# AlexandraLJones/MCBRaT3D

Hardware: AMD Instinct MI355X
Metric: photons/sec (higher is better)
Workload: dtype f32/f64

## Files before the change

mcbrat3d_amd/csrc/mcbrat_blockwalk.hip:

```cpp
#include <float.h>

#include "mcbrat_device.h"

namespace mcbrat {

enum : int { BW_DEAD = 0, BW_MOVE = 1, BW_COLLIDE = 2, BW_SURFACE = 3, BW_TOP = 4, BW_CROSS = 5 };

__device__ __forceinline__ int locate_z(const double *ze, int nz, bool regular, double z0, double invDz, double z) {
  if (!regular) return find_cell(ze, nz, z);
  return min(max((int)((z - z0) * invDz), 0), nz - 1);
}
__device__ __forceinline__ int locate_near_uniform(const double *e, int n, double x0, double invCell, double v) {
  int i = min(max((int)((v - x0) * invCell), 0), n - 1);
  const double lo = e[i], hi = e[i + 1];
  i += (v >= hi && i < n - 1) ? 1 : 0;
  i -= (v < lo && i > 0) ? 1 : 0;
  return i;
}

__device__ __forceinline__ long long unwrapped_index(const double *e, int n, double x0, double L, double invL, double x) {
  const double k = floor((x - x0) * invL);
  return (long long)k * n + find_cell(e, n, x - k * L);
}

struct BlockLds {
  size_t slab, cursor, rec, cdf, ext, ssa, cum, pfi, blockOf, tbl, total;
};
__host__ __device__ inline BlockLds block_lds_layout(int nx, int ny, int nz, int nc, size_t slabLen, int nBlocks, size_t tblFloats,
                                                      int optics = 0, bool cdfTop = false) {
  BlockLds L;
  const size_t nvox = (size_t)nx * ny * nz;
  const size_t nB4 = ((size_t)nBlocks + 3) & ~(size_t)3;
  size_t o = sizeof(double) * (size_t)(nx + ny + nz + 3);
  L.slab = o; o += sizeof(long long) * slabLen;
  L.cursor = o; o += 16;
  o = (o + 15) & ~(size_t)15;
  L.rec = o; o += 16 * (size_t)nBlocks;
  L.cdf = o; o += cdfTop ? sizeof(double) * ((size_t)nz + (size_t)ny * nz) : 0;
  L.ext = o; o += optics == 0 ? 4 * nvox : 4 * nB4;
  L.ssa = o; o += optics == 0 ? 4 * nvox * nc : (optics == 2 ? 4 * nB4 * nc : 0);
  L.cum = o; o += nc > 1 ? (optics == 0 ? 4 * nvox * nc : (optics == 2 ? 4 * nB4 * nc : 0)) : 0;
  L.pfi = o; o += optics == 0 ? 2 * ((nvox * nc + 1) & ~(size_t)1) : (optics == 2 ? 2 * nB4 * nc : 0);
  L.blockOf = o; o += 2 * ((nvox + 1) & ~(size_t)1);
  o = (o + 3) & ~(size_t)3;
  L.tbl = o; o += 4 * tblFloats;
  L.total = o;
  return L;
}

template <int BLOCK, bool TBL_LDS, bool DEBUG, bool EMIT, int SIMPLE, int OPT = 0>
__global__ void __launch_bounds__(BLOCK, BLOCK == 1024 ? 4 : (BLOCK > 512 ? BLOCK / 128 : MCBRAT_MIN_WAVES_PER_SIMD))
trace_block_kernel(const DevParams p) {
  constexpr bool NOY = SIMPLE == 2 && !DEBUG;
  constexpr bool NEAR = SIMPLE == 3;
  const bool xyRegular = NEAR ? false : (SIMPLE != 0 ? true : p.xyRegular != 0);
  const bool zRegular = NEAR ? false : (SIMPLE != 0 ? true : p.zRegular != 0);
  const int nc = SIMPLE != 0 ? 1 : p.nc;
  extern __shared__ __align__(16) unsigned char smem_raw[];
#ifdef MCBRAT_POISON
  for (unsigned i = threadIdx.x; i < p.ldsBytes / 4u; i += BLOCK) reinterpret_cast<unsigned *>(smem_raw)[i] = 0xffffffffu;
  __syncthreads();
#endif
  double *s_edge = reinterpret_cast<double *>(smem_raw);
  const int nEdges = p.nx + p.ny + p.nz + 3;
  const int ncol = p.nx * p.ny;
  const int nvox = ncol * p.nz;
  const int slabLen = (int)p.slabStride;
  const int slabsLen = p.unitsWide ? 2 * slabLen : slabLen;
  const bool cdfTop = EMIT && p.cdfTopLds != 0;
  const BlockLds lay = block_lds_layout(p.nx, p.ny, p.nz, nc, (size_t)slabsLen, p.nBlocks, TBL_LDS ? (size_t)p.tblTotalFloats : 0, OPT, cdfTop);
  const int nB4 = (p.nBlocks + 3) & ~3;
  long long *s_slab = reinterpret_cast<long long *>(smem_raw + lay.slab);
  unsigned *s_cursor = reinterpret_cast<unsigned *>(smem_raw + lay.cursor);
  uint4 *s_blockRec = reinterpret_cast<uint4 *>(smem_raw + lay.rec);
  float *s_ext = reinterpret_cast<float *>(smem_raw + lay.ext);
  double *s_cdfLevel = reinterpret_cast<double *>(smem_raw + lay.cdf);
  double *s_cdfRow = s_cdfLevel + p.nz;
  float *s_ssa = reinterpret_cast<float *>(smem_raw + lay.ssa);
  float *s_cum = reinterpret_cast<float *>(smem_raw + lay.cum);
  uint16_t *s_pfi = reinterpret_cast<uint16_t *>(smem_raw + lay.pfi);
  uint16_t *s_blockOf = reinterpret_cast<uint16_t *>(smem_raw + lay.blockOf);
  float *s_tbl = reinterpret_cast<float *>(smem_raw + lay.tbl);
  __shared__ int s_tblOffset[MCBRAT_MAX_COMPONENTS], s_tblNSteps[MCBRAT_MAX_COMPONENTS];
  __shared__ float s_tblInvN[MCBRAT_MAX_COMPONENTS];
  if (threadIdx.x < MCBRAT_MAX_COMPONENTS) {
    s_tblOffset[threadIdx.x] = p.tblOffset[threadIdx.x];
    s_tblNSteps[threadIdx.x] = p.tblNSteps[threadIdx.x];
    s_tblInvN[threadIdx.x] = p.tblInvN[threadIdx.x];
  }
  for (int i = threadIdx.x; i < nEdges; i += BLOCK) s_edge[i] = p.edges[i];
  if (TBL_LDS)
    for (int i = threadIdx.x; i < p.tblTotalFloats; i += BLOCK) s_tbl[i] = p.tables[i];
  for (int i = threadIdx.x; i < slabsLen; i += BLOCK) s_slab[i] = 0;
  if (threadIdx.x == 0) s_cursor[0] = 0;
  for (int i = threadIdx.x; i < p.nBlocks; i += BLOCK) s_blockRec[i] = p.blockRec[i];
  for (int i = threadIdx.x; i < nvox; i += BLOCK) s_blockOf[i] = p.blockOf[i];
  if (OPT == 0) {
    for (int i = threadIdx.x; i < nvox; i += BLOCK) s_ext[i] = p.ext[i];
    for (int i = threadIdx.x; i < nc * nvox; i += BLOCK) { s_ssa[i] = p.ssa[i]; s_pfi[i] = p.pfi[i]; }
    if (nc > 1)
      for (int i = threadIdx.x; i < nc * nvox; i += BLOCK) s_cum[i] = p.cum[i];
  } else {
    for (int i = threadIdx.x; i < p.nBlocks; i += BLOCK) s_ext[i] = p.blockExt[i];
    if (OPT == 2) {
      for (int i = threadIdx.x; i < nc * nB4; i += BLOCK) {
        const int k = i / nB4, b = i - k * nB4;
        if (b < p.nBlocks) { s_ssa[i] = p.blockSsa[k * p.nBlocks + b]; s_pfi[i] = p.blockPfi[k * p.nBlocks + b]; if (nc > 1) s_cum[i] = p.blockCum[k * p.nBlocks + b]; }
      }
    }
  }
  if (cdfTop) {
    const long long nxy = (long long)p.nx * p.ny;
    for (int i = threadIdx.x; i < p.nz; i += BLOCK) s_cdfLevel[i] = p.voxelCDF[((long long)p.nx - 1) + (long long)p.nx * (p.ny - 1) + nxy * i];
    for (int i = threadIdx.x; i < p.ny * p.nz; i += BLOCK) { const int k = i / p.ny, j = i - k * p.ny; s_cdfRow[i] = p.voxelCDF[((long long)p.nx - 1) + (long long)p.nx * j + nxy * k]; }
  }
  __syncthreads();
  auto cumAt = [&](int k, int cell) -> float { if constexpr (OPT == 0) return s_cum[k * nvox + cell]; else if constexpr (OPT == 1) return p.cum[k * nvox + cell]; else return s_cum[k * nB4 + s_blockOf[cell]]; };
  auto ssaAt = [&](int k, int cell) -> float { if constexpr (OPT == 0) return s_ssa[k * nvox + cell]; else if constexpr (OPT == 1) return p.ssa[k * nvox + cell]; else return s_ssa[k * nB4 + s_blockOf[cell]]; };
  auto pfiAt = [&](int k, int cell) -> int { if constexpr (OPT == 0) return (int)s_pfi[k * nvox + cell]; else if constexpr (OPT == 1) return (int)p.pfi[k * nvox + cell]; else return (int)s_pfi[k * nB4 + s_blockOf[cell]]; };
  auto extOfCell = [&](int cell) -> float { if constexpr (OPT == 0) return s_ext[cell]; else return s_ext[s_blockOf[cell]]; };
  const float *__restrict__ tbl = TBL_LDS ? s_tbl : p.tables;
  const int offY = p.nx + 1, offZ = p.nx + p.ny + 2;
  const double invDz = (double)p.nz / (p.zMax - p.z0);

  const int lane = threadIdx.x & (kWave - 1);
  const unsigned long long laneBelow = (1ull << lane) - 1ull;

  unsigned long long unitFirst = 0;
  unsigned unitCount = 0, unitSplit = 0;
  long long *unitSlab = nullptr;

  int state = BW_DEAD;
  bool more = true;
  int slabOff = 0;
  uint32_t idLo = 0, idHi = 0, event = 0;
  double px = 0, py = 0, pz = 0;
  float dx = 0, dy = 0, dz = 1;
  float ivx = 0, ivy = 0, ivz = 0;
  float tnx = 0, tny = 0, tnz = 0, tcur = 0;
  float acc = 0, tau = 0, w = 0, extCur = 0, uX = 0, uY = 0, uZ = 0;
  unsigned rx = 0, ry = 0, rz = 0;
  unsigned spans = 0;
  int nScat = 0, nLegs = 0;
  long long dbgX = 0, dbgY = 0;
  int dbgZ = 0;
  unsigned int cLegs = 0, cCross = 0, cColl = 0, cAbs = 0, cTop = 0, cSurf = 0, cKill = 0, cSurv = 0;
  unsigned long long wIters = 0, wCrossPhases = 0, wCrossLanes = 0, wEventLanes = 0, wLaunchPhases = 0, wSurfPhases = 0;

  auto countCrossings = [&](double x, double y, int kzEnd) {
    const long long ex = unwrapped_index(s_edge, p.nx, p.x0, p.Lx, p.invLx, x);
    const long long ey = unwrapped_index(s_edge + offY, p.ny, p.y0, p.Ly, p.invLy, y);
    cCross += (unsigned)(llabs(ex - dbgX) + llabs(ey - dbgY) + abs(kzEnd - dbgZ));
  };

  auto locX = [&](double xw, bool canLeave, bool force = false) {
    if (p.nx == 1 && !force) return 0;
    if (canLeave) {
      const double shift = floor((xw - p.x0) * p.invLx) * p.Lx;
      px -= shift; xw -= shift;
      if (DEBUG) dbgX -= (long long)rint(shift * p.invLx) * p.nx;
    }
    if (xyRegular) return min(max((int)((xw - p.x0) * p.invDX), 0), p.nx - 1);
    double o = 0.0;
    return locate_periodic(s_edge, p.nx, p.x0, p.Lx, p.invLx, p.invCellX, NEAR || p.xyNearUniform != 0, o, xw);
  };
  auto locY = [&](double yw, bool canLeave, bool force = false) {
    if (NOY) return 0;
    if (p.ny == 1 && !force) return 0;
    if (canLeave) {
      const double shift = floor((yw - p.y0) * p.invLy) * p.Ly;
      py -= shift; yw -= shift;
      if (DEBUG) dbgY -= (long long)rint(shift * p.invLy) * p.ny;
    }
    if (xyRegular) return min(max((int)((yw - p.y0) * p.invDY), 0), p.ny - 1);
    double o = 0.0;
    return locate_periodic(s_edge + offY, p.ny, p.y0, p.Ly, p.invLy, p.invCellY, NEAR || p.xyNearUniform != 0, o, yw);
  };
  auto inRange = [](int j, unsigned r) { return min(max(j, (int)(r & 0xffffu)), (int)(r >> 16) - 1); };
  const bool legacyNoClamp = (DEBUG || kTestBounds) && (p.legacyTies & 1) != 0, legacyMoveNaN = (DEBUG || kTestBounds) && (p.legacyTies & 2) != 0,
             legacyKeepSpans = (DEBUG || kTestBounds) && (p.legacyTies & 4) != 0;
  auto inRangeX = [&](int j, unsigned r) { return legacyNoClamp ? j : inRange(j, r); };
  auto enterBlock = [&](int ix, int iy, int iz) {
    const int cell = ix + p.nx * (iy + p.ny * iz);
    const unsigned blk = s_blockOf[cell];
    const uint4 rec = s_blockRec[blk];
    if constexpr (OPT == 0) extCur = s_ext[cell]; else extCur = s_ext[blk];
    rx = rec.x; rz = rec.z;
    if (!NOY) ry = rec.y;
    const int fx = dx >= 0.0f ? (int)(rx >> 16) : (int)(rx & 0xffffu);
    const int fy = NOY ? 0 : (dy >= 0.0f ? (int)(ry >> 16) : (int)(ry & 0xffffu));
    const int fz = dz >= 0.0f ? (int)(rz >> 16) : (int)(rz & 0xffffu);
    spans |= rec.w;
    tnx = ((rec.w & 1u) || ivx == 0.0f) ? FLT_MAX : (float)(s_edge[fx] - px) * ivx;
    tny = (NOY || (rec.w & 2u) || ivy == 0.0f) ? FLT_MAX : (float)(s_edge[offY + fy] - py) * ivy;
    tnz = ivz == 0.0f ? FLT_MAX : (float)(s_edge[offZ + fz] - pz) * ivz;
  };

  unsigned nCrossLeg = 0;
  unsigned nBadLane = 0;
  const unsigned maxEvents = (DEBUG || kTestBounds) ? p.maxEvents : kMaxEvents, maxEventsNaN = (DEBUG || kTestBounds) ? p.maxEventsNaN : kMaxEventsNaN,
                 watchdog = (DEBUG || kTestBounds) ? p.watchdog : kWatchdog;
#define MCBRAT_BW_DROP(kind_) do { \
    if constexpr (DEBUG || kTestBounds) record_first_drop(p.bad, (kind_), 2u, idLo, idHi, state, event);   \
    if (DEBUG && p.fates) p.fates[(((unsigned long long)idHi << 32) | idLo) - p.firstPhoton] = mcbrat_fate{3, 0, 0, 0, nScat, nLegs, w}; \
    state = BW_DEAD; \
    nBadLane = count_drop(nBadLane, (kind_));   \
  } while (0)
#ifdef MCBRAT_STAMPS
  __shared__ unsigned long long s_tprev[BLOCK / 64], s_stamp[BLOCK / 64][9];
  if (lane == 0) { s_tprev[threadIdx.x >> 6] = clock64(); for (int i = 0; i < 9; i++) s_stamp[threadIdx.x >> 6][i] = 0; }
#endif
  for (unsigned long long unit = blockIdx.x;; unit += gridDim.x) {
    if (unit >= p.nUnits) break;
    if (p.unitsWide) {
      const unsigned long long lo = p.total * unit / p.nUnits, hi = p.total * (unit + 1) / p.nUnits;
      const unsigned long long b = lo / p.ppb, end = (b + 1) * p.ppb;
      unitFirst = lo;
      unitCount = (unsigned)(hi - lo);
      unitSplit = (unsigned)((hi < end ? hi : end) - lo);
      unitSlab = p.slabs + b * p.slabStride;
    } else {
      const unsigned long long b = unit / p.unitsPerBatch, s = unit % p.unitsPerBatch;
      const unsigned long long bp = (p.total - b * p.ppb) < p.ppb ? (p.total - b * p.ppb) : p.ppb;
      const unsigned long long lo = (bp * s) / p.unitsPerBatch, hi = (bp * (s + 1)) / p.unitsPerBatch;
      unitFirst = b * p.ppb + lo;
      unitCount = (unsigned)(hi - lo);
      unitSplit = unitCount;
      unitSlab = p.slabs + b * p.slabStride;
    }
    more = true;

    for (;;) {
      bool needLeg = false;
      int ix = 0, iy = 0, iz = 0;

      const unsigned long long mSurf = __ballot(state == BW_SURFACE || state == BW_TOP);
      const unsigned long long mCross = __ballot(state == BW_CROSS);
      const int nBusy = __popcll(__ballot(state == BW_COLLIDE));
      const bool idle = nBusy < p.eventThreshold;
      const bool doSurface = __popcll(mSurf) >= p.surfaceThreshold || idle;
      const bool doCross = __popcll(mCross) >= p.crossThreshold || idle;
      if ((state == BW_SURFACE || state == BW_TOP) && doSurface) {
        const bool top = state == BW_TOP;
        {
          const double xw = px + (double)tcur * (double)dx, yw = py + (double)tcur * (double)dy;
          if (DEBUG) countCrossings(xw, yw, top ? p.nz : -1);
          px = xw;
          if (!NOY) py = yw;
          const int jx = locX(xw, true, true);
          ix = inRange(jx, rx);
          if (ix != jx) {
            const double lo = s_edge[rx & 0xffffu], hi = s_edge[rx >> 16];
            if (px < lo && lo - px > px + p.Lx - hi) px += p.Lx;
            else if (px > hi && px - hi > lo - (px - p.Lx)) px -= p.Lx;
          }
          iy = 0;
          if (!NOY) {
            const int jy = locY(yw, true, true);
            iy = inRange(jy, ry);
            if (iy != jy) {
              const double lo = s_edge[offY + (ry & 0xffffu)], hi = s_edge[offY + (ry >> 16)];
              if (py < lo && lo - py > py + p.Ly - hi) py += p.Ly;
              else if (py > hi && py - hi > lo - (py - p.Ly)) py -= p.Ly;
            }
          }
        }
        atomicAdd(reinterpret_cast<unsigned long long *>(s_slab + slabOff + (top ? 0 : ncol) + (ix + p.nx * iy)), weight_to_fixed(w));
        if (top) {
          if (DEBUG) {
            cTop++;
            if (p.fates) p.fates[(((unsigned long long)idHi << 32) | idLo) - p.firstPhoton] = mcbrat_fate{0, ix + 1, iy + 1, p.nz + 1, nScat, nLegs, w};
          }
          state = BW_DEAD;
        } else {
          pz = p.zSurf;
          iz = 0;
          nScat++;
          if (DEBUG) cSurf++;
          float mu = sqrtf(uX);
          if (!(fabsf(mu) > 2.0f * FLT_MIN)) {
            mu = sqrtf(uZ);
            uint32_t r[4];
            for (uint32_t j = 0; !(fabsf(mu) > 2.0f * FLT_MIN); j++) {
              if ((j & 3u) == 0) philox4x32_10(event, 2u + (j >> 2), idLo, idHi, p.seedLo, p.seedHi, r);
              mu = sqrtf(u01(pick4(r, j & 3u)));
            }
          }
          const float wIn = w;
          if (SIMPLE == 0 && p.surfNumX > 0) w = w * surface_reflectance(p, px, py);
          else w = (float)((double)w * (double)p.albedo);
          if (w <= FLT_MIN) {
            if (DEBUG && p.fates) p.fates[(((unsigned long long)idHi << 32) | idLo) - p.firstPhoton] = mcbrat_fate{1, ix + 1, iy + 1, 1, nScat, nLegs, wIn};
            state = BW_DEAD;
          } else {
            const float sinTheta = sqrtf(1.0f - mu * mu);
            float cphi, sphi;
            sincos_2pi(uY, cphi, sphi);
            dx = sinTheta * cphi; dy = sinTheta * sphi; dz = mu;
            needLeg = true;
          }
        }
      }
      STAMP(5);
      const unsigned long long mDead = __ballot(state == BW_DEAD && more);
      const bool doLaunch = __popcll(mDead) >= p.launchThreshold || idle;
      const unsigned long long want = doLaunch ? mDead : 0ull;
      if (DEBUG) {
        wIters++;
        wEventLanes += nBusy;
        if (want) wLaunchPhases++;
        if (doSurface && mSurf) wSurfPhases++;
        if (doCross && mCross) { wCrossPhases++; wCrossLanes += __popcll(mCross); }
      }
      if (want != 0ull) {
        const int nWant = __popcll(want);
        const int rank = __popcll(want & laneBelow);
        unsigned base = 0;
        if (lane == 0) base = atomicAdd(&s_cursor[0], (unsigned)nWant);
        base = (unsigned)__shfl((int)base, 0);
        const unsigned k = base + (unsigned)rank;
        const bool valid = k < unitCount;
        const unsigned long long myIdx = unitFirst + k;
        if (state == BW_DEAD && more) {
          if (valid) {
            const unsigned long long id = p.firstPhoton + myIdx;
            idLo = (uint32_t)id; idHi = (uint32_t)(id >> 32);
            event = 0; nScat = 0; nLegs = 0;
            slabOff = k < unitSplit ? 0 : slabLen;
            uint32_t r[4];
            philox4x32_10(0u, 0u, idLo, idHi, p.seedLo, p.seedHi, r);
            double lx, ly, lz;
            if (!EMIT) {
              lx = (double)u01(r[0]);
              ly = (double)u01(r[1]);
              lz = 0.0;
              dx = p.dir0[0]; dy = p.dir0[1]; dz = p.dir0[2];
            } else {
              float mu = 0.f, phi = 0.f;
              const float sel = u01(r[0]);
              if ((double)sel > p.fracAtms) {
                lx = (double)u01(r[1]);
                ly = (double)u01(r[2]);
                lz = 0.0;
                uint32_t r1[4];
                for (uint32_t j = 0;; j++) {
                  if ((j & 3u) == 0) philox4x32_10(0u, 1u + (j >> 2), idLo, idHi, p.seedLo, p.seedHi, r1);
                  mu = sqrtf(u01(pick4(r1, j & 3u)));
                  if (fabsf(mu) > 2.0f * FLT_MIN) break;
                }
                phi = (u01(r[3]) * 2.0f) * 3.14159274f;
              } else {
                const float rn = u01(r[1]);
                const long long nxy = (long long)p.nx * p.ny;
                const int ik = cdfTop ? find_cdf(s_cdfLevel, p.nz, 1, rn) : find_cdf(p.voxelCDF + ((long long)p.nx - 1) + (long long)p.nx * (p.ny - 1), p.nz, nxy, rn);
                const int ij = cdfTop ? find_cdf(s_cdfRow + p.ny * (ik - 1), p.ny, 1, rn) : find_cdf(p.voxelCDF + ((long long)p.nx - 1) + nxy * (ik - 1), p.ny, p.nx, rn);
                const int ii = find_cdf(p.voxelCDF + (long long)p.nx * ((ij - 1) + (long long)p.ny * (ik - 1)), p.nx, 1, rn);
                uint32_t r1[4];
                philox4x32_10(0u, 1u, idLo, idHi, p.seedLo, p.seedHi, r1);
                lz = ((double)(ik - 1) * 1.0 / (double)p.nz) + (double)(u01(r[2]) / (float)p.nz);
                if (ik == 1 && lz == 0.0) lz = 2.220446049250313e-16;
                if (ik == p.nz && lz > 1.0 - 2.0 * 2.220446049250313e-16) lz = lz - 2.0 * 2.220446049250313e-16;
                lx = ((double)(ii - 1) * 1.0 / (double)p.nx) + (double)(u01(r[3]) * (1.0f / (float)p.nx));
                ly = ((double)(ij - 1) * 1.0 / (double)p.ny) + (double)(u01(r1[0]) * (1.0f / (float)p.ny));
                uint32_t r2[4];
                for (uint32_t j = 0;; j++) {
                  uint32_t uu;
                  if (j < 2) uu = j ? r1[3] : r1[2];
                  else {
                    if (((j - 2) & 3u) == 0) philox4x32_10(0u, 2u + ((j - 2) >> 2), idLo, idHi, p.seedLo, p.seedHi, r2);
                    uu = pick4(r2, (j - 2) & 3u);
                  }
                  mu = 1.0f - (2.0f * u01(uu));
                  if (fabsf(mu) > 2.0f * FLT_MIN) break;
                }
                phi = (u01(r1[1]) * 2.0f) * 3.14159274f;
              }
              const float sinTheta = sqrtf(1.0f - mu * mu);
              dx = sinTheta * cosf(phi); dy = sinTheta * sinf(phi); dz = mu;
            }
            w = 1.0f;
            px = p.x0 + lx * (p.xMax - p.x0);
            if (!NOY) py = p.y0 + ly * (p.yMax - p.y0);
            if (xyRegular) {
              ix = min((int)((px - p.x0) * p.invDX), p.nx - 1);
              iy = NOY ? 0 : min((int)((py - p.y0) * p.invDY), p.ny - 1);
            } else {
              ix = NEAR ? locate_near_uniform(s_edge, p.nx, p.x0, p.invCellX, px) : find_cell(s_edge, p.nx, px);
              iy = NOY ? 0 : (NEAR ? locate_near_uniform(s_edge + offY, p.ny, p.y0, p.invCellY, py) : find_cell(s_edge + offY, p.ny, py));
            }
            if (!EMIT) {
              pz = p.zLaunch; iz = p.izLaunch;
            } else if (zRegular) {
              pz = p.z0 + lz * (p.zMax - p.z0);
              iz = min((int)((pz - p.z0) / ((p.zMax - p.z0) / (double)p.nz)), p.nz - 1);
            } else {
              const double t = (lz - p.z0) * (double)p.nz;
              const double fl = floor(t);
              iz = min((int)fl, p.nz - 1);
              pz = s_edge[offZ + iz] + (t - fl) * (s_edge[offZ + iz + 1] - s_edge[offZ + iz]);
            }
            if (EMIT && p.lwFlag && pz > 0.0)
              atomicAdd(reinterpret_cast<unsigned long long *>(s_slab + slabOff + 2 * ncol + (ix + p.nx * (iy + p.ny * iz))), to_fixed(-1.0));
            needLeg = true;
          } else {
            more = false;
          }
        }
      }
      STAMP(0);
      if (state == BW_COLLIDE) {
        if (dz == dz || legacyMoveNaN) {
          const double s = (double)(tcur + div_fast(tau - acc, extCur));
          px = px + s * (double)dx;
          if (!NOY) py = py + s * (double)dy;
          pz = pz + s * (double)dz;
        }
        {
          const double xw = px, yw = py;
          iz = NEAR ? locate_near_uniform(s_edge + offZ, p.nz, p.z0, invDz, pz) : locate_z(s_edge + offZ, p.nz, zRegular, p.z0, invDz, pz);
          ix = locX(xw, (spans & 1u) != 0);
          iy = locY(yw, (spans & 2u) != 0);
        }
        int cell = ix + p.nx * (iy + p.ny * iz);
        nScat++;
        if (DEBUG) cColl++;
        int c = 0;
        if (nc > 1) {
          for (int k = 0; k < nc - 1; k++)
            if (uZ >= cumAt(k, cell)) c = k + 1;
        }
        float ssa = ssaAt(c, cell);
        int pfEntry = pfiAt(c, cell);
        if (ssa <= 0.0f && extOfCell(cell) != extCur) {
          ix = inRange(ix, rx); iz = inRange(iz, rz);
          if (!NOY) iy = inRange(iy, ry);
          cell = ix + p.nx * (iy + p.ny * iz);
          c = 0;
          if (nc > 1) {
            for (int k = 0; k < nc - 1; k++)
              if (uZ >= cumAt(k, cell)) c = k + 1;
          }
          ssa = ssaAt(c, cell);
          pfEntry = pfiAt(c, cell);
        }
        if (DEBUG) countCrossings(px, py, iz);
        if (ssa < 1.0f) {
          atomicAdd(reinterpret_cast<unsigned long long *>(s_slab + slabOff + 2 * ncol + cell), weight_to_fixed(w * (1.0f - ssa)));
          w = w * ssa;
          if (DEBUG) cAbs++;
        }
        if (p.useRR && w < 0.5f) {
          float uR = uZ;
          if (nc != 1) {
            uint32_t r1[4];
            philox4x32_10(event, 1u, idLo, idHi, p.seedLo, p.seedHi, r1);
            uR = u01(r1[1]);
          }
          if (uR >= w) { w = 0.0f; if (DEBUG) cKill++; }
          else { w = 1.0f; if (DEBUG) cSurv++; }
        }
        STAMP(2);
        if (w <= FLT_MIN) {
          if (DEBUG && p.fates) p.fates[(((unsigned long long)idHi << 32) | idLo) - p.firstPhoton] = mcbrat_fate{2, ix + 1, iy + 1, iz + 1, nScat, nLegs, 0.0f};
          state = BW_DEAD;
        } else {
          const int n = s_tblNSteps[c];
          const float *t = tbl + s_tblOffset[c] + (long long)pfEntry * n;
          const int ai = (int)(uX * (float)n) + 1;
          float ang;
          if (ai < n) {
#ifdef MCBRAT_PRECISE_MATH
            const float left = uX - (float)(ai - 1) / (float)n;
#else
            const float left = uX - (float)(ai - 1) * s_tblInvN[c];
#endif
            ang = (1.0f - left) * t[ai - 1] + left * t[ai];
          } else {
            ang = t[n - 1];
          }
#ifdef MCBRAT_PRECISE_MATH
          const float cs = cosf(ang);
#else
          const float cs = cos_0_pi(ang);
#endif
          STAMP(3);
          float AX, AY;
          sincos_2pi(uY, AX, AY);
#ifdef MCBRAT_PRECISE_MATH
          float B = sqrtf(1.0f - cs * cs);
#else
          float B = __builtin_amdgcn_sqrtf(1.0f - cs * cs);
#endif
          AX = AX * B;
          AY = AY * B;
          B = dx * AX - dy * AY;
          float D = cs - div_fast(B, 1.0f + fabsf(dz));
          dx = dx * D + AX;
          dy = dy * D - AY;
          dz = dz * cs - copysignf(fabsf(B), dz * B);
          needLeg = true;
          STAMP(4);
        }
      }
      STAMP(4);
      if (needLeg && event >= maxEventsNaN) {
        if (event >= maxEvents || !(dz == dz || w < 1.0f)) { needLeg = false; MCBRAT_BW_DROP(event >= maxEvents ? DROP_LEGS : DROP_NAN_LEGS); }
      }
      if (needLeg) {
        event++;
        nLegs++;
        if (DEBUG) {
          cLegs++;
          dbgX = unwrapped_index(s_edge, p.nx, p.x0, p.Lx, p.invLx, px);
          dbgY = unwrapped_index(s_edge + offY, p.ny, p.y0, p.Ly, p.invLy, py);
          dbgZ = iz;
        }
        uint32_t r[4];
        philox4x32_10(event, 0u, idLo, idHi, p.seedLo, p.seedHi, r);
#ifdef MCBRAT_PRECISE_MATH
        tau = -logf(fmaxf(FLT_MIN, u01(r[0])));
#else
        tau = -0.693147182f * __builtin_amdgcn_logf(fmaxf(FLT_MIN, u01(r[0])));
#endif
        uX = u01(r[1]); uY = u01(r[2]); uZ = u01(r[3]);
        acc = 0.0f; tcur = 0.0f;
        ivx = fabsf(dx) >= 2.0f * FLT_MIN ? rcp_fast(dx) : 0.0f;
        ivy = (!NOY && fabsf(dy) >= 2.0f * FLT_MIN) ? rcp_fast(dy) : 0.0f;
        ivz = fabsf(dz) >= 2.0f * FLT_MIN ? rcp_fast(dz) : 0.0f;
        spans = 0;
        nCrossLeg = 0u;
        enterBlock(ix, iy, iz);
        state = BW_MOVE;
      }
      STAMP(6);
      if (state == BW_CROSS && doCross) {
        const bool yLtX = !NOY && tny < tnx;
        const float m2 = yLtX ? tny : tnx;
        const bool isZ = tnz < m2;
        const double xw = px + (double)tcur * (double)dx, yw = py + (double)tcur * (double)dy, zw = pz + (double)tcur * (double)dz;
        int jx, jy, jz;
        if (isZ) {
          jz = dz >= 0.0f ? (int)(rz >> 16) : (int)(rz & 0xffffu) - 1;
          jx = inRangeX(locX(xw, (spans & 1u) != 0), rx);
          jy = NOY ? 0 : inRangeX(locY(yw, (spans & 2u) != 0), ry);
        } else if (yLtX) {
          jy = dy >= 0.0f ? (int)(ry >> 16) : (int)(ry & 0xffffu) - 1;
          if (jy >= p.ny) { jy = 0; py -= p.Ly; if (DEBUG) dbgY -= p.ny; }
          else if (jy < 0) { jy = p.ny - 1; py += p.Ly; if (DEBUG) dbgY += p.ny; }
          jx = inRangeX(locX(xw, (spans & 1u) != 0), rx);
          jz = inRangeX(NEAR ? locate_near_uniform(s_edge + offZ, p.nz, p.z0, invDz, zw) : locate_z(s_edge + offZ, p.nz, zRegular, p.z0, invDz, zw), rz);
        } else {
          jx = dx >= 0.0f ? (int)(rx >> 16) : (int)(rx & 0xffffu) - 1;
          if (jx >= p.nx) { jx = 0; px -= p.Lx; if (DEBUG) dbgX -= p.nx; }
          else if (jx < 0) { jx = p.nx - 1; px += p.Lx; if (DEBUG) dbgX += p.nx; }
          jy = NOY ? 0 : inRangeX(locY(yw, (spans & 2u) != 0), ry);
          jz = inRangeX(NEAR ? locate_near_uniform(s_edge + offZ, p.nz, p.z0, invDz, zw) : locate_z(s_edge + offZ, p.nz, zRegular, p.z0, invDz, zw), rz);
        }
        if (!legacyKeepSpans) spans = 0;
        enterBlock(jx, jy, jz);
        state = BW_MOVE;
        if (++nCrossLeg > watchdog) MCBRAT_BW_DROP(DROP_CROSSINGS);
      }
      STAMP(1);
      if (__ballot(state != BW_DEAD || more) == 0ull) break;

#ifdef MCBRAT_STUCK_PROBE
      if (DEBUG && p.traceBuf && wIters > 3000000ull) {
        const unsigned long long live = __ballot(state != BW_DEAD);
        if (live != 0ull && lane == __ffsll((long long)live) - 1) {
          const unsigned long long r = wIters - 3000001ull;
          if (r < 64ull) {
            double *t = p.traceBuf + 20 * r;
            t[0] = 777; t[1] = state; t[2] = tcur; t[3] = tnx; t[4] = tny; t[5] = tnz; t[6] = (double)rx; t[7] = (double)ry; t[8] = (double)rz;
            t[9] = px; t[10] = py; t[11] = pz; t[12] = dx; t[13] = dy; t[14] = dz; t[15] = acc; t[16] = tau; t[17] = extCur; t[18] = spans; t[19] = idLo;
          } else {
            state = BW_DEAD;
          }
        }
      }
#endif
      if (state == BW_MOVE) {
        const bool yLtX = !NOY && tny < tnx;
        const float m2 = yLtX ? tny : tnx;
        const bool isZ = tnz < m2;
        const float tmin = isZ ? tnz : m2;
        const float accNew = acc + (tmin - tcur) * extCur;
        if (accNew > tau) {
          state = BW_COLLIDE;
        } else if (!(tmin < FLT_MAX)) {
          MCBRAT_BW_DROP(DROP_VACUUM);
        } else {
          acc = accNew;
          tcur = tmin;
          state = BW_CROSS;
          if (isZ && (dz >= 0.0f ? (int)(rz >> 16) == p.nz : (rz & 0xffffu) == 0u)) state = dz >= 0.0f ? BW_TOP : BW_SURFACE;
        }
      }
      STAMP(7);
    }

    __syncthreads();
    for (int i = threadIdx.x; i < slabsLen; i += BLOCK) {
      const long long v = s_slab[i];
      if (v != 0) {
        atomicAdd(reinterpret_cast<unsigned long long *>(unitSlab + i), (unsigned long long)v);
        s_slab[i] = 0;
      }
    }
    if (threadIdx.x == 0) s_cursor[0] = 0;
    __syncthreads();
  }

  publish_drops(p.bad, nBadLane);
#ifdef MCBRAT_STAMPS
  if (DEBUG && p.counters && lane == 0) for (int i = 0; i < 9; i++) atomicAdd(p.counters + 16 + i, s_stamp[threadIdx.x >> 6][i]);
#endif
  if (DEBUG && p.counters) {
    atomicAdd(p.counters + 0, (unsigned long long)cLegs);
    atomicAdd(p.counters + 1, (unsigned long long)cCross);
    atomicAdd(p.counters + 2, (unsigned long long)cColl);
    atomicAdd(p.counters + 3, (unsigned long long)cAbs);
    atomicAdd(p.counters + 4, (unsigned long long)cTop);
    atomicAdd(p.counters + 5, (unsigned long long)cSurf);
    atomicAdd(p.counters + 6, (unsigned long long)cKill);
    atomicAdd(p.counters + 7, (unsigned long long)cSurv);
    if (lane == 0) {
      atomicAdd(p.counters + 8, wCrossPhases); atomicAdd(p.counters + 9, wCrossLanes);
      atomicAdd(p.counters + 10, wIters); atomicAdd(p.counters + 11, wEventLanes);
      atomicAdd(p.counters + 12, wLaunchPhases); atomicAdd(p.counters + 13, wSurfPhases);
    }
  }
}

}
```

mcbrat3d_amd/csrc/mcbrat_kernels.hip:

```cpp
#include <float.h>

#include "mcbrat_device.h"

#ifdef MCBRAT_STAMPS
#define STAMP(i) do { if (DEBUG && p.counters) { const unsigned long long t_ = clock64(); \
    if (lane == __ffsll((long long)__ballot(1)) - 1) { s_stamp[threadIdx.x >> 6][i] += t_ - s_tprev[threadIdx.x >> 6]; s_tprev[threadIdx.x >> 6] = t_; } } } while (0)
#elif defined(MCBRAT_MARKS)
#define STAMP(i) asm volatile("; @@mark " #i)
#else
#define STAMP(i) do { } while (0)
#endif

namespace mcbrat {

constexpr unsigned kChunk = 256;
#ifndef MCBRAT_FLY_MIN_BRICKS
#define MCBRAT_FLY_MIN_BRICKS 8.0f
#endif
constexpr float kFlyMinBricks = MCBRAT_FLY_MIN_BRICKS;
constexpr int kWalkCap = 256;

#ifndef MCBRAT_MIN_WAVES_PER_SIMD
#define MCBRAT_MIN_WAVES_PER_SIMD 4
#endif
#ifndef MCBRAT_WAVES_GLOBAL_GRID
#define MCBRAT_WAVES_GLOBAL_GRID 6
#endif
#ifndef MCBRAT_WAVES_GLOBAL_GRID_INTEN
#define MCBRAT_WAVES_GLOBAL_GRID_INTEN 4
#endif

__device__ __forceinline__ uint32_t xor3(uint32_t a, uint32_t b, uint32_t c) {
#if defined(__gfx950__)
  return __builtin_amdgcn_bitop3_b32(a, b, c, 0x96);
#else
  return a ^ b ^ c;
#endif
}

__device__ __forceinline__ void philox4x32_10(uint32_t c0, uint32_t c1, uint32_t c2, uint32_t c3, uint32_t k0,
                                              uint32_t k1, uint32_t (&out)[4]) {
#pragma unroll
  for (int i = 0; i < 10; i++) {
    const unsigned long long p0 = (unsigned long long)0xD2511F53u * c0;
    const unsigned long long p1 = (unsigned long long)0xCD9E8D57u * c2;
    c0 = xor3((uint32_t)(p1 >> 32), c1, k0);
    c1 = (uint32_t)p1;
    c2 = xor3((uint32_t)(p0 >> 32), c3, k1);
    c3 = (uint32_t)p0;
    k0 += 0x9E3779B9u;
    k1 += 0xBB67AE85u;
  }
  out[0] = c0; out[1] = c1; out[2] = c2; out[3] = c3;
}

__device__ __forceinline__ float u01(uint32_t u) { return (float)u * 2.3283064365386963e-10f; }

#ifdef MCBRAT_PRECISE_MATH
__device__ __forceinline__ float rcp_fast(float x) { return 1.0f / x; }
__device__ __forceinline__ float div_fast(float a, float b) { return a / b; }
#else
__device__ __forceinline__ float rcp_fast(float x) { return __builtin_amdgcn_rcpf(x); }
__device__ __forceinline__ float div_fast(float a, float b) { return a * __builtin_amdgcn_rcpf(b); }
#endif

__device__ __forceinline__ float cos_0_pi(float x) {
  const float q = rintf(x * 0.636619772f);
  float r = __fmaf_rn(q, -1.57079637050628662109375f, x);
  r = __fmaf_rn(q, 4.371138828673793e-8f, r);
  const float z = r * r;
  const float c = __fmaf_rn(z, __fmaf_rn(z, __fmaf_rn(z, __fmaf_rn(z, 2.43904487962774090654e-5f, -1.38867637746099294692e-3f),
                                                      4.16666233237390631894e-2f), -0.499999997251031003120f), 1.0f);
  const float s = __fmaf_rn(r * z, __fmaf_rn(z, __fmaf_rn(z, __fmaf_rn(z, 2.7183114939898219064e-6f, -1.98393348360966317347e-4f),
                                                          8.3333293858894631756e-3f), -0.166666666416265235595f), r);
  return q == 0.0f ? c : (q == 1.0f ? -s : -c);
}

__device__ __forceinline__ void sincos_2pi(float u, float &c, float &s) {
  const float q = rintf(4.0f * u);
  const float r = (u - 0.25f * q) * 6.28318548202514648f;
  const float z = r * r;
  const float cc = __fmaf_rn(z, __fmaf_rn(z, __fmaf_rn(z, __fmaf_rn(z, 2.43904487962774090654e-5f, -1.38867637746099294692e-3f),
                                                       4.16666233237390631894e-2f), -0.499999997251031003120f), 1.0f);
  const float ss = __fmaf_rn(r * z, __fmaf_rn(z, __fmaf_rn(z, __fmaf_rn(z, 2.7183114939898219064e-6f, -1.98393348360966317347e-4f),
                                                           8.3333293858894631756e-3f), -0.166666666416265235595f), r);
  const int qi = (int)q & 3;
  c = qi == 0 ? cc : (qi == 1 ? -ss : (qi == 2 ? -cc : ss));
  s = qi == 0 ? ss : (qi == 1 ? cc : (qi == 2 ? -ss : -cc));
}

__device__ __forceinline__ uint32_t pick4(const uint32_t (&r)[4], uint32_t i) {
  const uint32_t a = (i & 1u) ? r[1] : r[0], b = (i & 1u) ? r[3] : r[2];
  return (i & 2u) ? b : a;
}

__device__ __forceinline__ unsigned long long to_fixed(double v) {
  return (unsigned long long)__double2ll_rn(v * kTallyScale);
}
__device__ __forceinline__ unsigned long long weight_to_fixed(float v) {
  return v >= 1.0f ? (1ull << 32) : (unsigned long long)__float2uint_rn(v * 4294967296.0f);
}

__device__ __forceinline__ int find_cell(const double *e, int n, double v) {
  int lo = 0, hi = n;
  while (hi - lo > 1) {
    const int mid = (lo + hi) >> 1;
    if (v >= e[mid]) lo = mid; else hi = mid;
  }
  return lo;
}

__device__ __forceinline__ int find_cdf(const double *t, int n, long long stride, float vf) {
  const double v = (double)vf;
  int lo = 0, hi = n;
  while (!(lo == n || hi <= lo + 1)) {
    const int mid = (lo + hi) >> 1;
    if (v > t[(long long)(mid - 1) * stride]) lo = mid; else hi = mid;
  }
  return hi;
}

__device__ __forceinline__ int locate_periodic(const double *e, int n, double x0, double L, double invL, double invCell,
                                               bool nearUniform, double &origin, double xw) {
  const double shift = floor((xw - x0) * invL) * L;
  origin -= shift;
  xw -= shift;
  if (!nearUniform) return find_cell(e, n, xw);
  int i = min(max((int)((xw - x0) * invCell), 0), n - 1);
  const double lo = e[i], hi = e[i + 1];
  i += (xw >= hi && i < n - 1) ? 1 : 0;
  i -= (xw < lo && i > 0) ? 1 : 0;
  return i;
}

__device__ __forceinline__ float make_periodic_f(double a, double aMin, double aMax) {
  float r = (float)a;
  for (int guard = 0; guard < 65536; ++guard) {
    if ((double)r <= aMax && (double)r > aMin) break;
    if ((double)r > aMax) r = (float)((double)r - (aMax - aMin));
    else if ((double)r == aMin) r = (float)aMax;
    else r = (float)((double)r + (aMax - aMin));
  }
  return r;
}
__device__ __forceinline__ int find_index_mixed(const double *t, int n, float vf) {
  const double v = (double)vf;
  int lo = 0, up = n;
  while (!(lo == n || up <= lo + 1)) {
    const int mid = (lo + up) >> 1;
    if (v >= t[mid - 1]) lo = mid; else up = mid;
  }
  return lo;
}
__device__ __forceinline__ float surface_reflectance(const DevParams &p, double x, double y) {
  const int xi = min(max(find_index_mixed(p.surfX, p.surfNumX, make_periodic_f(x, p.surfX[0], p.surfX[p.surfNumX - 1])), 1), p.surfNumX - 1);
  const int yi = min(max(find_index_mixed(p.surfY, p.surfNumY, make_periodic_f(y, p.surfY[0], p.surfY[p.surfNumY - 1])), 1), p.surfNumY - 1);
  return p.surfRefl[(xi - 1) + (p.surfNumX - 1) * (yi - 1)];
}

struct CellRef {
  int dense;
  int stored;
};

template <bool BRICK>
__device__ __forceinline__ CellRef locate_cell(const DevParams &p, int ix, int iy, int iz) {
  CellRef r;
  r.dense = ix + p.nx * (iy + p.ny * iz);
  r.stored = -1;
  if (BRICK) {
    const uint32_t base = p.brickTable[(ix >> 2) + p.nbx * ((iy >> 2) + p.nby * (iz >> 2))];
    if (base != 0xffffffffu) r.stored = (int)(base + (uint32_t)((ix & 3) + 4 * ((iy & 3) + 4 * (iz & 3))));
  }
  return r;
}

template <bool BRICK>
__device__ __forceinline__ float load_ext(const DevParams &p, const float *s_bgExt, const CellRef &r, int iz) {
  if (!BRICK) return p.extWalk[r.dense];
  return r.stored >= 0 ? p.ext[r.stored] : s_bgExt[iz];
}

template <int BLOCK, bool TBL_LDS, int PRIV, bool BRICK, bool DEBUG, bool INTEN = false, bool EMIT = true, int SPEC = 0>
__global__ void __launch_bounds__(BLOCK, BLOCK == 1024 ? 4 : BLOCK > 512 ? BLOCK / 128 : ((PRIV == 0 && !DEBUG) ? (INTEN ? MCBRAT_WAVES_GLOBAL_GRID_INTEN : MCBRAT_WAVES_GLOBAL_GRID) : MCBRAT_MIN_WAVES_PER_SIMD))
trace_kernel(const DevParams p) {
  constexpr int WALKSPEC = SPEC & 3, NCSPEC = (SPEC >> 2) & 3;
  static_assert(SPEC == 0 || WALKSPEC != 0, "the component count and the roulette are fixed in the walk-specialised instantiations only");
  const bool layerSkipOn = SPEC ? true : p.layerSkip != 0;
  const bool useRec = SPEC ? true : p.rec != nullptr;
  const bool xyRegularWalk = (WALKSPEC == 2 || WALKSPEC == 3) ? true : (WALKSPEC == 1 ? false : p.xyRegularWalk != 0);
  const bool zRegularWalk = WALKSPEC == 2 ? true : ((WALKSPEC == 1 || WALKSPEC == 3) ? false : p.zRegularWalk != 0);
  const bool surfaceDescription = SPEC ? false : p.surfNumX > 0;
  const int nc = NCSPEC ? NCSPEC : p.nc;
  const bool useRR = (SPEC & 16) ? true : p.useRR != 0;
  extern __shared__ __align__(16) unsigned char smem_raw[];
#ifdef MCBRAT_POISON
  for (unsigned i = threadIdx.x; i < p.ldsBytes / 4u; i += BLOCK) reinterpret_cast<unsigned *>(smem_raw)[i] = 0xffffffffu;
  __syncthreads();
#endif
  double *s_edge = reinterpret_cast<double *>(smem_raw);
  const int nEdges = p.nx + p.ny + p.nz + 3;
  const int offZ0 = p.nx + p.ny + 2;
  const int ncol = p.nx * p.ny;
  const int slabLen = PRIV ? (int)p.slabStride : 0;
  long long *s_slab = reinterpret_cast<long long *>(s_edge + nEdges);
  unsigned *s_cursor = reinterpret_cast<unsigned *>(s_slab + slabLen);
  float *s_bgExt = reinterpret_cast<float *>(s_cursor + (PRIV ? 4 : 0));
  constexpr bool gridLds = PRIV == 2;
  const int nvoxS = gridLds ? ncol * p.nz : 0;
  int *s_run = reinterpret_cast<int *>(s_bgExt + ((p.nz + 3) & ~3));
  double *s_runT = reinterpret_cast<double *>(s_run + ((p.nz + 3) & ~3));
  constexpr bool FLY = PRIV != 2 && !BRICK && !INTEN;
  const bool flyOn = FLY && (SPEC ? true : p.fly != 0);
  const int flyCols = FLY ? p.flyNbx * p.flyNby : 0;
  float *s_bgVal = reinterpret_cast<float *>(s_runT + ((p.nz + 2) & ~1));
  float2 *s_rangeZ = reinterpret_cast<float2 *>(s_bgVal + (flyCols ? ((p.nz + 3) & ~3) : 0));
  uint16_t *s_range = reinterpret_cast<uint16_t *>(s_rangeZ + flyCols);
  float *s_ext = reinterpret_cast<float *>(s_range + ((flyCols + 3) & ~3));
  float *s_ssa = s_ext + nvoxS;
  float *s_cum = s_ssa + (size_t)nc * nvoxS;
  uint16_t *s_pfi = reinterpret_cast<uint16_t *>(s_cum + (size_t)nc * nvoxS);
  float *s_tbl = reinterpret_cast<float *>(s_pfi + (((size_t)nc * nvoxS + 1) & ~(size_t)1));
  __shared__ int s_tblOffset[MCBRAT_MAX_COMPONENTS], s_tblNSteps[MCBRAT_MAX_COMPONENTS];
  __shared__ float s_tblInvN[MCBRAT_MAX_COMPONENTS];
  __shared__ int s_fwdOffset[MCBRAT_MAX_COMPONENTS], s_fwdNAngles[MCBRAT_MAX_COMPONENTS];
  __shared__ float s_flyTC[(PRIV != 2 && !BRICK && !INTEN) ? BLOCK : 1];
  if (INTEN && threadIdx.x < MCBRAT_MAX_COMPONENTS) {
    s_fwdOffset[threadIdx.x] = p.fwdOffset[threadIdx.x];
    s_fwdNAngles[threadIdx.x] = p.fwdNAngles[threadIdx.x];
  }
  if (threadIdx.x < MCBRAT_MAX_COMPONENTS) {
    s_tblOffset[threadIdx.x] = p.tblOffset[threadIdx.x];
    s_tblNSteps[threadIdx.x] = p.tblNSteps[threadIdx.x];
    s_tblInvN[threadIdx.x] = p.tblInvN[threadIdx.x];
  }
  for (int i = threadIdx.x; i < nEdges; i += BLOCK) s_edge[i] = p.edges[i];
  if (TBL_LDS)
    for (int i = threadIdx.x; i < p.tblTotalFloats; i += BLOCK) s_tbl[i] = p.tables[i];
  if (PRIV) {
    for (int i = threadIdx.x; i < slabLen; i += BLOCK) s_slab[i] = 0;
    if (threadIdx.x == 0) s_cursor[0] = 0;
  }
  for (int i = threadIdx.x; i < p.nz; i += BLOCK) { s_bgExt[i] = p.bgExt[i]; s_run[i] = p.layerRun[i]; }
  for (int i = threadIdx.x; i <= p.nz; i += BLOCK) s_runT[i] = p.layerRunT[i];
  if (FLY && flyCols) {
    for (int i = threadIdx.x; i < p.nz; i += BLOCK) s_bgVal[i] = p.bgVal[i];
    for (int i = threadIdx.x; i < flyCols; i += BLOCK) {
      const unsigned r = p.flyRange[i];
      s_range[i] = (uint16_t)r;
      s_rangeZ[i] = make_float2((float)p.edges[offZ0 + (r & 0xffu)], (float)p.edges[offZ0 + (r >> 8)]);
    }
  }
  if (gridLds) {
    for (int i = threadIdx.x; i < nvoxS; i += BLOCK) s_ext[i] = p.ext[i];
    for (int i = threadIdx.x; i < nc * nvoxS; i += BLOCK) { s_ssa[i] = p.ssa[i]; s_cum[i] = p.cum[i]; s_pfi[i] = p.pfi[i]; }
  }
  __syncthreads();
  const float *__restrict__ tbl = TBL_LDS ? s_tbl : p.tables;
  const int offY = p.nx + 1, offZ = p.nx + p.ny + 2;
  typedef const float __attribute__((address_space(1))) *GlobalFloats;
  GlobalFloats extG = (GlobalFloats)p.extWalk;
  const float zTopF = (float)p.zMax, zBotF = (float)p.z0;
  if constexpr (!INTEN) asm volatile("" : "+s"(extG));

  const int lane = threadIdx.x & (kWave - 1);
  const unsigned long long laneBelow = (1ull << lane) - 1ull;

  unsigned long long unitFirst = 0;
  unsigned unitCount = 0;
  long long *unitSlab = nullptr;

  int state = ST_DEAD;
  bool more = true;
  uint32_t idLo = 0, idHi = 0, event = 0, batch = 0;
  double px = 0, py = 0, pz = 0;
  float dx = 0, dy = 0, dz = 1;
  float ivx = 0, ivy = 0, ivz = 0;
  float tnx = 0, tny = 0, tnz = 0, tcur = 0;
  float acc = 0, tau = 0, w = 0, extCur = 0, uX = 0, uY = 0, uZ = 0;
  int ex = 0, ey = 0, ez = 0;
  int cell = 0;
  int pendCell = -1;
  unsigned long long pendDep = 0ull;
  unsigned nBadLane = 0;
#define MCBRAT_FLUSH_PENDING() do { if (!PRIV && pendCell >= 0) { \
    atomicAdd(reinterpret_cast<unsigned long long *>(p.slabs + (unsigned long long)batch * p.slabStride + 2 * ncol + pendCell), pendDep); pendCell = -1; } } while (0)
#define MCBRAT_DROP_PHOTON(kind_) do { \
    if constexpr (DEBUG || kTestBounds) record_first_drop(p.bad, (kind_), 1u, idLo, idHi, state, event);   \
    if (DEBUG && p.fates) p.fates[(((unsigned long long)idHi << 32) | idLo) - p.firstPhoton] = mcbrat_fate{3, 0, 0, 0, nScat, nLegs, w}; \
    MCBRAT_FLUSH_PENDING(); \
    state = ST_DEAD; \
    nBadLane = count_drop(nBadLane, (kind_));   \
  } while (0)
  constexpr bool LAZY = PRIV != 2 && !BRICK;
  bool lazy = false;
  double dbgU0 = 0, dbgV0 = 0;
  int stride = 1;
  bool noFly = false;
  bool flyToCollision = false;
  int dbgK0 = 0;
  int brickId = -1;
  uint32_t brickBase = 0xffffffffu;
  int nScat = 0, nLegs = 0;
  int iFlag = 0, iEntry = 0;
  float iW = 0, iDx = 0, iDy = 0, iDz = 0;
  unsigned long long chunkNext = 0, chunkEnd = 0;
  unsigned int cLegs = 0, cCross = 0, cColl = 0, cAbs = 0, cTop = 0, cSurf = 0, cKill = 0, cSurv = 0;
#ifdef MCBRAT_STAMPS
  __shared__ unsigned long long s_tprev[BLOCK / 64], s_stamp[BLOCK / 64][9];
  if (lane == 0) { s_tprev[threadIdx.x >> 6] = clock64(); for (int i = 0; i < 9; i++) s_stamp[threadIdx.x >> 6][i] = 0; }
#endif
  unsigned long long wWalkIters = 0, wWalkLanes = 0, wEventPhases = 0, wEventLanes = 0, wLaunchPhases = 0, wSurfPhases = 0;

  auto tryJump = [&]() {
    const bool up = dz >= 0.0f;
    const int k = ez - offZ - (up ? 1 : 0);
    const int run = s_run[k];
    const int fEnd = up ? (run >> 16) : (run & 0xffff);
    const double dT = up ? s_runT[fEnd] - s_runT[k + 1] : s_runT[k] - s_runT[fEnd];
    extCur = fabsf(extCur);
    const float accEnd = acc + (tnz - tcur) * extCur + (float)dT * fabsf(ivz);
    if (DEBUG) { dbgU0 = (px + (double)tcur * (double)dx - p.x0) * p.invCellX; dbgV0 = (py + (double)tcur * (double)dy - p.y0) * p.invCellY; }
    lazy = true;
    tnx = FLT_MAX; tny = FLT_MAX;
    state = ST_WALK;
    if (accEnd <= tau) {
      acc = accEnd;
      tcur = (float)(s_edge[offZ + fEnd] - pz) * ivz;
      if (DEBUG) cCross += (unsigned)(up ? fEnd - k : k + 1 - fEnd);
      if (up) { ez = offZ + fEnd + 1; state = fEnd == p.nz ? ST_TOP : ST_ENTER; }
      else { ez = offZ + fEnd - 1; state = fEnd == 0 ? ST_SURFACE : ST_ENTER; }
      if (state == ST_SURFACE) extCur = s_bgExt[0];
      tnz = (float)(s_edge[min(max(ez, offZ), offZ + p.nz)] - pz) * ivz;
    }
  };
  auto resolveXY = [&]() {
    const float tc = state == ST_COLLIDE ? tcur + div_fast(tau - acc, fabsf(extCur)) : tcur;
    const double xw = px + (double)tc * (double)dx, yw = py + (double)tc * (double)dy;
    if (DEBUG) cCross += (unsigned)(fabs(floor((xw - p.x0) * p.invCellX) - floor(dbgU0)) + fabs(floor((yw - p.y0) * p.invCellY) - floor(dbgV0)));
    const int jx = locate_periodic(s_edge, p.nx, p.x0, p.Lx, p.invLx, p.invCellX, p.xyNearUniform != 0, px, xw);
    const int jy = locate_periodic(s_edge + offY, p.ny, p.y0, p.Ly, p.invLy, p.invCellY, p.xyNearUniform != 0, py, yw);
    ex = jx + (dx >= 0.0f ? 1 : 0);
    ey = offY + jy + (dy >= 0.0f ? 1 : 0);
    tnx = ivx != 0.0f ? (float)(s_edge[ex] - px) * ivx : FLT_MAX;
    tny = ivy != 0.0f ? (float)(s_edge[ey] - py) * ivy : FLT_MAX;
    cell = jx + p.nx * (jy + p.ny * (ez - offZ - (dz >= 0.0f ? 1 : 0)));
    lazy = false;
    if (state == ST_ENTER) { extCur = extG[cell]; state = ST_WALK; noFly = false; }
  };
  auto tryFly = [&]() -> bool {
    const bool up = dz >= 0.0f;
    const int k = ez - offZ - (up ? 1 : 0);
    const int jx = ex - (dx >= 0.0f ? 1 : 0), jy = ey - offY - (dy >= 0.0f ? 1 : 0);
    const double zw = pz + (double)tcur * (double)dz;
    const double Tz = s_runT[k] + (double)s_bgVal[k] * (zw - s_edge[offZ + k]);
    const float dT = (float)((up ? s_runT[p.nz] : 0.0) - Tz) * ivz;
// ... 1174 lines not shown
```

Measured before the change: 5.566 billion.

## Precompute per-photon Philox product, use mbcnt ranks, umul24 cell indexing, branchless move

Caches the first-round Philox multiply of the photon id per photon so each RNG call skips one 64-bit product. Replaces the per-lane 'more' flag with a wave-uniform mask, and computes launch ranks with mbcnt intrinsics plus inverse_ballot. Uses 24-bit multiplies for cell and table indexing, hoists the edge-distance conversions, and makes the MOVE state transition branchless. Together these aim to cut scalar and vector ALU work in the hot walk loop. They add a 64-bit register per lane, and umul24 assumes grid and table indices fit in 24 bits.

```diff
diff --git a/mcbrat3d_amd/csrc/mcbrat_blockwalk.hip b/mcbrat3d_amd/csrc/mcbrat_blockwalk.hip
--- a/mcbrat3d_amd/csrc/mcbrat_blockwalk.hip
+++ b/mcbrat3d_amd/csrc/mcbrat_blockwalk.hip
@@ -124,16 +124,16 @@
   const double invDz = (double)p.nz / (p.zMax - p.z0);
 
   const int lane = threadIdx.x & (kWave - 1);
-  const unsigned long long laneBelow = (1ull << lane) - 1ull;
 
   unsigned long long unitFirst = 0;
   unsigned unitCount = 0, unitSplit = 0;
   long long *unitSlab = nullptr;
 
   int state = BW_DEAD;
-  bool more = true;
+  unsigned long long moreMask = ~0ull;
   int slabOff = 0;
   uint32_t idLo = 0, idHi = 0, event = 0;
+  unsigned long long idP1 = 0;
   double px = 0, py = 0, pz = 0;
   float dx = 0, dy = 0, dz = 1;
   float ivx = 0, ivy = 0, ivz = 0;
@@ -180,8 +180,13 @@
   const bool legacyNoClamp = (DEBUG || kTestBounds) && (p.legacyTies & 1) != 0, legacyMoveNaN = (DEBUG || kTestBounds) && (p.legacyTies & 2) != 0,
              legacyKeepSpans = (DEBUG || kTestBounds) && (p.legacyTies & 4) != 0;
   auto inRangeX = [&](int j, unsigned r) { return legacyNoClamp ? j : inRange(j, r); };
+  const unsigned nx24 = (unsigned)p.nx, ncol24 = (unsigned)ncol;
+  auto cellOf = [&](int ix, int iy, int iz) -> int {
+    if (NOY) return ix + (int)__umul24(ncol24, (unsigned)iz);
+    return ix + (int)__umul24(nx24, (unsigned)(iy + (int)__umul24((unsigned)p.ny, (unsigned)iz)));
+  };
   auto enterBlock = [&](int ix, int iy, int iz) {
-    const int cell = ix + p.nx * (iy + p.ny * iz);
+    const int cell = cellOf(ix, iy, iz);
     const unsigned blk = s_blockOf[cell];
     const uint4 rec = s_blockRec[blk];
     if constexpr (OPT == 0) extCur = s_ext[cell]; else extCur = s_ext[blk];
@@ -191,9 +196,10 @@
     const int fy = NOY ? 0 : (dy >= 0.0f ? (int)(ry >> 16) : (int)(ry & 0xffffu));
     const int fz = dz >= 0.0f ? (int)(rz >> 16) : (int)(rz & 0xffffu);
     spans |= rec.w;
-    tnx = ((rec.w & 1u) || ivx == 0.0f) ? FLT_MAX : (float)(s_edge[fx] - px) * ivx;
+    const float ex = (float)(s_edge[fx] - px), ez = (float)(s_edge[offZ + fz] - pz);
+    tnx = ((rec.w & 1u) || ivx == 0.0f) ? FLT_MAX : ex * ivx;
     tny = (NOY || (rec.w & 2u) || ivy == 0.0f) ? FLT_MAX : (float)(s_edge[offY + fy] - py) * ivy;
-    tnz = ivz == 0.0f ? FLT_MAX : (float)(s_edge[offZ + fz] - pz) * ivz;
+    tnz = ivz == 0.0f ? FLT_MAX : ez * ivz;
   };
 
   unsigned nCrossLeg = 0;
@@ -228,7 +234,7 @@
       unitSplit = unitCount;
       unitSlab = p.slabs + b * p.slabStride;
     }
-    more = true;
+    moreMask = ~0ull;
 
     for (;;) {
       bool needLeg = false;
@@ -282,7 +288,7 @@
             mu = sqrtf(uZ);
             uint32_t r[4];
             for (uint32_t j = 0; !(fabsf(mu) > 2.0f * FLT_MIN); j++) {
-              if ((j & 3u) == 0) philox4x32_10(event, 2u + (j >> 2), idLo, idHi, p.seedLo, p.seedHi, r);
+              if ((j & 3u) == 0) philox4x32_10_p1(event, 2u + (j >> 2), idP1, idHi, p.seedLo, p.seedHi, r);
               mu = sqrtf(u01(pick4(r, j & 3u)));
             }
           }
@@ -302,7 +308,7 @@
         }
       }
       STAMP(5);
-      const unsigned long long mDead = __ballot(state == BW_DEAD && more);
+      const unsigned long long mDead = __ballot(state == BW_DEAD) & moreMask;
       const bool doLaunch = __popcll(mDead) >= p.launchThreshold || idle;
       const unsigned long long want = doLaunch ? mDead : 0ull;
       if (DEBUG) {
@@ -314,21 +320,23 @@
       }
       if (want != 0ull) {
         const int nWant = __popcll(want);
-        const int rank = __popcll(want & laneBelow);
+        const unsigned rank = __builtin_amdgcn_mbcnt_hi((unsigned)(want >> 32), __builtin_amdgcn_mbcnt_lo((unsigned)want, 0u));
         unsigned base = 0;
         if (lane == 0) base = atomicAdd(&s_cursor[0], (unsigned)nWant);
         base = (unsigned)__shfl((int)base, 0);
-        const unsigned k = base + (unsigned)rank;
+        const unsigned k = base + rank;
         const bool valid = k < unitCount;
         const unsigned long long myIdx = unitFirst + k;
-        if (state == BW_DEAD && more) {
+        const unsigned long long mValid = __ballot(valid);
+        if (__builtin_amdgcn_inverse_ballot_w64(want)) {
           if (valid) {
             const unsigned long long id = p.firstPhoton + myIdx;
             idLo = (uint32_t)id; idHi = (uint32_t)(id >> 32);
+            idP1 = philox_p1(idLo);
             event = 0; nScat = 0; nLegs = 0;
             slabOff = k < unitSplit ? 0 : slabLen;
             uint32_t r[4];
-            philox4x32_10(0u, 0u, idLo, idHi, p.seedLo, p.seedHi, r);
+            philox4x32_10_p1(0u, 0u, idP1, idHi, p.seedLo, p.seedHi, r);
             double lx, ly, lz;
             if (!EMIT) {
               lx = (double)u01(r[0]);
@@ -344,7 +352,7 @@
                 lz = 0.0;
                 uint32_t r1[4];
                 for (uint32_t j = 0;; j++) {
-                  if ((j & 3u) == 0) philox4x32_10(0u, 1u + (j >> 2), idLo, idHi, p.seedLo, p.seedHi, r1);
+                  if ((j & 3u) == 0) philox4x32_10_p1(0u, 1u + (j >> 2), idP1, idHi, p.seedLo, p.seedHi, r1);
                   mu = sqrtf(u01(pick4(r1, j & 3u)));
                   if (fabsf(mu) > 2.0f * FLT_MIN) break;
                 }
@@ -356,7 +364,7 @@
                 const int ij = cdfTop ? find_cdf(s_cdfRow + p.ny * (ik - 1), p.ny, 1, rn) : find_cdf(p.voxelCDF + ((long long)p.nx - 1) + nxy * (ik - 1), p.ny, p.nx, rn);
                 const int ii = find_cdf(p.voxelCDF + (long long)p.nx * ((ij - 1) + (long long)p.ny * (ik - 1)), p.nx, 1, rn);
                 uint32_t r1[4];
-                philox4x32_10(0u, 1u, idLo, idHi, p.seedLo, p.seedHi, r1);
+                philox4x32_10_p1(0u, 1u, idP1, idHi, p.seedLo, p.seedHi, r1);
                 lz = ((double)(ik - 1) * 1.0 / (double)p.nz) + (double)(u01(r[2]) / (float)p.nz);
                 if (ik == 1 && lz == 0.0) lz = 2.220446049250313e-16;
                 if (ik == p.nz && lz > 1.0 - 2.0 * 2.220446049250313e-16) lz = lz - 2.0 * 2.220446049250313e-16;
@@ -367,7 +375,7 @@
                   uint32_t uu;
                   if (j < 2) uu = j ? r1[3] : r1[2];
                   else {
-                    if (((j - 2) & 3u) == 0) philox4x32_10(0u, 2u + ((j - 2) >> 2), idLo, idHi, p.seedLo, p.seedHi, r2);
+                    if (((j - 2) & 3u) == 0) philox4x32_10_p1(0u, 2u + ((j - 2) >> 2), idP1, idHi, p.seedLo, p.seedHi, r2);
                     uu = pick4(r2, (j - 2) & 3u);
                   }
                   mu = 1.0f - (2.0f * u01(uu));
@@ -402,10 +410,9 @@
             if (EMIT && p.lwFlag && pz > 0.0)
               atomicAdd(reinterpret_cast<unsigned long long *>(s_slab + slabOff + 2 * ncol + (ix + p.nx * (iy + p.ny * iz))), to_fixed(-1.0));
             needLeg = true;
-          } else {
-            more = false;
-          }
-        }
+          }
+        }
+        moreMask &= ~want | mValid;
       }
       STAMP(0);
       if (state == BW_COLLIDE) {
@@ -421,7 +428,7 @@
           ix = locX(xw, (spans & 1u) != 0);
           iy = locY(yw, (spans & 2u) != 0);
         }
-        int cell = ix + p.nx * (iy + p.ny * iz);
+        int cell = cellOf(ix, iy, iz);
         nScat++;
         if (DEBUG) cColl++;
         int c = 0;
@@ -434,7 +441,7 @@
         if (ssa <= 0.0f && extOfCell(cell) != extCur) {
           ix = inRange(ix, rx); iz = inRange(iz, rz);
           if (!NOY) iy = inRange(iy, ry);
-          cell = ix + p.nx * (iy + p.ny * iz);
+          cell = cellOf(ix, iy, iz);
           c = 0;
           if (nc > 1) {
             for (int k = 0; k < nc - 1; k++)
@@ -453,7 +460,7 @@
           float uR = uZ;
           if (nc != 1) {
             uint32_t r1[4];
-            philox4x32_10(event, 1u, idLo, idHi, p.seedLo, p.seedHi, r1);
+            philox4x32_10_p1(event, 1u, idP1, idHi, p.seedLo, p.seedHi, r1);
             uR = u01(r1[1]);
           }
           if (uR >= w) { w = 0.0f; if (DEBUG) cKill++; }
@@ -465,7 +472,7 @@
           state = BW_DEAD;
         } else {
           const int n = s_tblNSteps[c];
-          const float *t = tbl + s_tblOffset[c] + (long long)pfEntry * n;
+          const float *t = tbl + s_tblOffset[c] + (TBL_LDS ? (long long)__umul24((unsigned)pfEntry, (unsigned)n) : (long long)pfEntry * n);
           const int ai = (int)(uX * (float)n) + 1;
           float ang;
           if (ai < n) {
@@ -516,7 +523,7 @@
           dbgZ = iz;
         }
         uint32_t r[4];
-        philox4x32_10(event, 0u, idLo, idHi, p.seedLo, p.seedHi, r);
+        philox4x32_10_p1(event, 0u, idP1, idHi, p.seedLo, p.seedHi, r);
 #ifdef MCBRAT_PRECISE_MATH
         tau = -logf(fmaxf(FLT_MIN, u01(r[0])));
 #else
@@ -562,7 +569,7 @@
         if (++nCrossLeg > watchdog) MCBRAT_BW_DROP(DROP_CROSSINGS);
       }
       STAMP(1);
-      if (__ballot(state != BW_DEAD || more) == 0ull) break;
+      if ((__ballot(state != BW_DEAD) | moreMask) == 0ull) break;
 
 #ifdef MCBRAT_STUCK_PROBE
       if (DEBUG && p.traceBuf && wIters > 3000000ull) {
@@ -585,16 +592,16 @@
         const bool isZ = tnz < m2;
         const float tmin = isZ ? tnz : m2;
         const float accNew = acc + (tmin - tcur) * extCur;
-        if (accNew > tau) {
-          state = BW_COLLIDE;
-        } else if (!(tmin < FLT_MAX)) {
+        const bool coll = accNew > tau;
+        const bool up = dz >= 0.0f;
+        const bool out = isZ && (up ? (int)(rz >> 16) == p.nz : (rz & 0xffffu) == 0u);
+        const int next = coll ? BW_COLLIDE : (out ? (up ? BW_TOP : BW_SURFACE) : BW_CROSS);
+        acc = coll ? acc : accNew;
+        tcur = coll ? tcur : tmin;
+        if (!coll && !(tmin < FLT_MAX))
           MCBRAT_BW_DROP(DROP_VACUUM);
-        } else {
-          acc = accNew;
-          tcur = tmin;
-          state = BW_CROSS;
-          if (isZ && (dz >= 0.0f ? (int)(rz >> 16) == p.nz : (rz & 0xffffu) == 0u)) state = dz >= 0.0f ? BW_TOP : BW_SURFACE;
-        }
+        else
+          state = next;
       }
       STAMP(7);
     }
diff --git a/mcbrat3d_amd/csrc/mcbrat_kernels.hip b/mcbrat3d_amd/csrc/mcbrat_kernels.hip
--- a/mcbrat3d_amd/csrc/mcbrat_kernels.hip
+++ b/mcbrat3d_amd/csrc/mcbrat_kernels.hip
@@ -52,6 +52,25 @@
     k1 += 0xBB67AE85u;
   }
   out[0] = c0; out[1] = c1; out[2] = c2; out[3] = c3;
+}
+
+__device__ __forceinline__ unsigned long long philox_p1(uint32_t c2) { return (unsigned long long)0xCD9E8D57u * c2; }
+__device__ __forceinline__ void philox4x32_10_p1(uint32_t c0, uint32_t c1, unsigned long long p1, uint32_t c3, uint32_t k0,
+                                                 uint32_t k1, uint32_t (&out)[4]) {
+  const unsigned long long p0 = (unsigned long long)0xD2511F53u * c0;
+  uint32_t d0 = xor3((uint32_t)(p1 >> 32), c1, k0), d1 = (uint32_t)p1, d2 = xor3((uint32_t)(p0 >> 32), c3, k1), d3 = (uint32_t)p0;
+#pragma unroll
+  for (int i = 1; i < 10; i++) {
+    k0 += 0x9E3779B9u;
+    k1 += 0xBB67AE85u;
+    const unsigned long long q0 = (unsigned long long)0xD2511F53u * d0;
+    const unsigned long long q1 = (unsigned long long)0xCD9E8D57u * d2;
+    d0 = xor3((uint32_t)(q1 >> 32), d1, k0);
+    d1 = (uint32_t)q1;
+    d2 = xor3((uint32_t)(q0 >> 32), d3, k1);
+    d3 = (uint32_t)q0;
+  }
+  out[0] = d0; out[1] = d1; out[2] = d2; out[3] = d3;
 }
 
 __device__ __forceinline__ float u01(uint32_t u) { return (float)u * 2.3283064365386963e-10f; }
```

Measured after the change: 5.768 billion (median of 6 runs). 3.6% higher.
